# atx/padne

Hardware: AMD Instinct MI355X
Metric: CG solves/s (higher is better)
Workload: dtype f64

## Files before the change

padne_amd/csrc/amg.hip:

```cpp
#include "common.hpp"

#include <functional>
#include <type_traits>
#include <memory>

#include <algorithm>
#include <chrono>
#include <math.h>
#include <stdlib.h>
#include <string.h>

namespace padne {

struct AmgLevel {
    const padne_csr *A = nullptr;
    padne_csr *A_owned = nullptr;
    padne_csr *P = nullptr;
    padne_csr *R = nullptr;
    padne_csr *W = nullptr;
    double lambda = 2.0;
    double jac = 0.0;
    long long n = 0;
    double *b = nullptr, *xa = nullptr, *xb = nullptr, *tmp = nullptr;
    float *b8 = nullptr, *xa8 = nullptr, *xb8 = nullptr, *tmp8 = nullptr;
// ... 18 lines not shown
    int *seg_off = nullptr;
    double *coarse_gather = nullptr;
    double *tail_r = nullptr, *tail_z = nullptr;
    int *tail_slot_idx = nullptr;
    double setup_seconds = 0.0;
    double operator_complexity = 0.0;
    int device = 0;
};

constexpr double kTheta = 0.08;
constexpr double kOmegaNum = 1.5;
constexpr double kChebRatio = 10.0;
constexpr int kLanczosSteps = 8;
constexpr int kMaxLevels = 16;

struct __attribute__((packed, aligned(4))) I4u { int x, y, z, w; };
struct __attribute__((packed, aligned(4))) I2u { int x, y; };
struct __attribute__((packed, aligned(4))) D2u { double x, y; };
struct __attribute__((packed, aligned(4))) L2u { long long x, y; };
__device__ __forceinline__ int4 load_i4_unaligned(const int *p) {
    const I4u v = *reinterpret_cast<const I4u *>(p);
    return make_int4(v.x, v.y, v.z, v.w);
}
__device__ __forceinline__ double2 load_d2_unaligned(const double *p) {
    const D2u v = *reinterpret_cast<const D2u *>(p);
    return make_double2(v.x, v.y);
}

template <int LANES>
__device__ __forceinline__ int scan_incl_lanes(int x) {
    x += __builtin_amdgcn_update_dpp(0, x, 0x111, 0xf, 0xf, false);
    x += __builtin_amdgcn_update_dpp(0, x, 0x112, 0xf, 0xf, false);
    x += __builtin_amdgcn_update_dpp(0, x, 0x114, 0xf, 0xf, false);
    x += __builtin_amdgcn_update_dpp(0, x, 0x118, 0xf, 0xf, false);
    if (LANES >= 32) x += __builtin_amdgcn_update_dpp(0, x, 0x142, 0xa, 0xf, false);
    if (LANES == 64) x += __builtin_amdgcn_update_dpp(0, x, 0x143, 0xc, 0xf, false);
    return x;
}

__device__ __forceinline__ unsigned xcd_bid() {
    const unsigned b = blockIdx.x, per = gridDim.x >> 3;
    if (b >= (per << 3)) return b;
    return (b & 7u) * per + (b >> 3);
}
struct XcdSweep { long long t0, t1, stride; };
__device__ __forceinline__ XcdSweep xcd_sweep(const long long n_tiles, const int waves_per_block, const int w) {
    const unsigned G = gridDim.x;
    const unsigned nslab = (G % kNumXcd == 0) ? kNumXcd : 1;
    const unsigned slab = blockIdx.x % nslab;
    XcdSweep sw;
    const long long s0 = (long long)slab * n_tiles / nslab;
    sw.t1 = (long long)(slab + 1) * n_tiles / nslab;
    sw.t0 = s0 + (long long)(blockIdx.x / nslab) * waves_per_block + w;
    sw.stride = (long long)(G / nslab) * waves_per_block;
    return sw;
}



constexpr unsigned int kMisRoot = 0xffffffffu;
__device__ __forceinline__ unsigned int prio32_of(int i) {
    unsigned int h = (unsigned int)i & 0x7fffffffu;
    h = (h * 0x5bd1e995u) & 0x7fffffffu;
    h ^= h >> 15;
    h = (h * 0x2c1b3c6du) & 0x7fffffffu;
    h ^= h >> 13;
    h = (h * 0x297a2d39u) & 0x7fffffffu;
    h ^= h >> 16;
    return h + 1u;
}

__device__ __forceinline__ bool strong(double a, double di, double dj, double theta2) {
    return a * a * di * dj >= theta2;
}

__device__ __forceinline__ int xw_position(const int4 d, const int run, const int c) {
    int pos = 0;
    if (c >= d.z && c < d.z + run) pos = 2 * run + (c - d.z);
    if (c >= d.y && c < d.y + run) pos = run + (c - d.y);
    if (c >= d.x && c < d.x + run) pos = c - d.x;
    return pos;
}

__global__ __launch_bounds__(256) void strength_mark(int n, int n_wtiles, const int *__restrict__ rowptr,
                                                     const int *__restrict__ cols, const double *__restrict__ vals,
                                                     const double *__restrict__ dinv, double theta2,
                                                     int *__restrict__ scol, double *__restrict__ bound_partial,
                                                     const int4 *__restrict__ xw_desc = nullptr,
                                                     const unsigned char *__restrict__ xw_lidx = nullptr,
                                                     const int xw_run = 0, unsigned char *__restrict__ spos = nullptr,
                                                     float *__restrict__ vals32 = nullptr) {
    constexpr int CH = 512;
    __shared__ unsigned char rid_all[4 * CH];
    __shared__ double pv_all[4 * CH];
    __shared__ double red[4], red2[4];
    const int lane = threadIdx.x & 63, w = threadIdx.x >> 6;
    unsigned char *rid = rid_all + w * CH;
    double *pv = pv_all + w * CH;
    const XcdSweep sw = xcd_sweep(n_wtiles, 4, w);
    double my_max = 0.0, my_plain = 0.0;
    for (long long wt = sw.t0; wt < sw.t1; wt += sw.stride) {
        const int row0 = (int)wt * 64;
        const int row1 = min(row0 + 64, n);
        const int r = row0 + lane;
        int rs = 0, re = 0;
        double di = 0.0;
        if (r < row1) {
            rs = rowptr[r];
            re = rowptr[r + 1];
            di = dinv[r];
        }
        const int k0 = __shfl(rs, 0, 64);
        const int k1 = __shfl(re, row1 - row0 - 1, 64);
        double dF = r < row1 ? 1.0 / di : 1.0, off_strong = 0.0, off_all = 0.0, abs_all = 0.0;
        int4 dsc = make_int4(0, 0, 0, 0);
        if (spos != nullptr) dsc = xw_desc[wt];
        const bool windowed = spos != nullptr && dsc.w != 0;
        const int self_pos = windowed ? xw_position(dsc, xw_run, r) : 0;
        for (int base = k0; base < k1; base += CH) {
            const int lo = max(rs, base), hi = min(re, base + CH);
            for (int k = lo; k < hi; ++k) rid[k - base] = (unsigned char)lane;
            asm volatile("s_waitcnt lgkmcnt(0)" ::: "memory");
            __builtin_amdgcn_wave_barrier();
#pragma unroll
            for (int q = 0; q < CH / 64; ++q) {
                const int e = base + lane + 64 * q;
                const int rl = e < k1 ? rid[e - base] : 0;
                const double dr = __shfl(di, rl, 64);
                const int sp = __shfl(self_pos, rl, 64);
                if (e < k1) {
                    const int i = row0 + rl;
                    const int c = cols[e];
                    const double v = vals[e];
                    if (vals32 != nullptr) vals32[e] = (float)v;
                    const bool st = c != i && strong(v, dr, dinv[c], theta2);
                    scol[e] = st ? c : i;
                    if (windowed) spos[e] = st ? xw_lidx[e] : (unsigned char)sp;
                    if (bound_partial != nullptr) {
                        rid[e - base] = (unsigned char)(rl | (c == i ? 0x40 : 0) | (st ? 0x80 : 0));
                        pv[e - base] = v;
                    }
                }
            }
            if (bound_partial != nullptr) {
                asm volatile("s_waitcnt lgkmcnt(0)" ::: "memory");
                __builtin_amdgcn_wave_barrier();
                for (int k = lo; k < hi; ++k) {
                    const unsigned char f = rid[k - base];
                    const double v = pv[k - base];
                    abs_all += fabs(v);
                    if (f & 0x40) continue;
                    off_all += fabs(v);
                    if (f & 0x80) off_strong += fabs(v);
                    else dF += v;
                }
            }
            asm volatile("" ::: "memory");
            __builtin_amdgcn_wave_barrier();
        }
        if (bound_partial != nullptr && r < row1) {
            double off = off_strong;
            if (!(dF * di > 0.05)) {
                dF = 1.0 / di;
                off = off_all;
            }
            const double sgm = (off + fabs(dF)) / fabs(dF);
            my_max = sgm > my_max ? sgm : my_max;
            const double plain = abs_all * fabs(di);
            my_plain = plain > my_plain ? plain : my_plain;
        }
    }
    if (bound_partial != nullptr) {
        for (int o = 32; o > 0; o >>= 1) {
            my_max = fmax(my_max, __shfl_down(my_max, o, 64));
            my_plain = fmax(my_plain, __shfl_down(my_plain, o, 64));
        }
        if (lane == 0) {
            red[w] = my_max;
            red2[w] = my_plain;
        }
        __syncthreads();
        if (threadIdx.x == 0) {
            bound_partial[blockIdx.x] = fmax(fmax(red[0], red[1]), fmax(red[2], red[3]));
            bound_partial[kMaxPartials + blockIdx.x] = fmax(fmax(red2[0], red2[1]), fmax(red2[2], red2[3]));
        }
    }
}

template <typename T>
__global__ __launch_bounds__(256) void nbr_max(int n, int n_wtiles, const int *__restrict__ srow,
                                               const int *__restrict__ scol, const T *__restrict__ in,
                                               T *__restrict__ out) {
    constexpr int CH = 512;
    __shared__ T park_all[4 * CH];
    const int lane = threadIdx.x & 63, w = threadIdx.x >> 6;
    T *park = park_all + w * CH;
    const XcdSweep sw = xcd_sweep(n_wtiles, 4, w);
    for (long long wt = sw.t0; wt < sw.t1; wt += sw.stride) {
        const int row0 = (int)wt * 64;
        const int row1 = min(row0 + 64, n);
        const int r = row0 + lane;
        int rs = 0, re = 0;
        T m = 0;
        if (r < row1) {
            rs = srow[r];
            re = srow[r + 1];
            m = in[r];
        }
        const int k0 = __shfl(rs, 0, 64);
        const int k1 = __shfl(re, row1 - row0 - 1, 64);
        for (int base = k0; base < k1; base += CH) {
#pragma unroll
            for (int j = 0; j < CH / 64; ++j) {
                const int e = base + lane + 64 * j;
                park[lane + 64 * j] = (e < k1) ? in[scol[e]] : (T)0;
            }
            asm volatile("s_waitcnt lgkmcnt(0)" ::: "memory");
            __builtin_amdgcn_wave_barrier();
            const int lo = max(rs, base), hi = min(re, base + CH);
            for (int k = lo; k < hi; ++k) {
                const T v = park[k - base];
                m = v > m ? v : m;
            }
            asm volatile("" ::: "memory");
            __builtin_amdgcn_wave_barrier();
        }
        if (r < row1) out[r] = m;
    }
}

template <typename T>
__global__ __launch_bounds__(256) void nbr_max_wpr(int n, const int *__restrict__ srow, const int *__restrict__ scol,
                                                   const T *__restrict__ in, T *__restrict__ out) {
    const int lane = threadIdx.x & 63;
    const long long r = (long long)blockIdx.x * 4 + (threadIdx.x >> 6);
    if (r >= n) return;
    const int rs = srow[r], re = srow[r + 1];
    T m = in[r];
    for (int k = rs + lane; k < re; k += 64) {
        const T v = in[scol[k]];
        m = v > m ? v : m;
    }
#pragma unroll
    for (int off = 32; off > 0; off >>= 1) {
        const T o = __shfl_down(m, off, 64);
        m = o > m ? o : m;
    }
    if (lane == 0) out[r] = m;
}

__device__ __forceinline__ bool mis_decide_one(int i, unsigned int top, unsigned int *__restrict__ word,
                                               signed char *__restrict__ state) {
    const unsigned int mine = word[i];
    if (top == kMisRoot) {
        state[i] = 2;
        word[i] = 0u;
        return false;
    }
    if (top == mine) {
        state[i] = 1;
        word[i] = kMisRoot;
        return false;
    }
    return true;
}

template <typename T, bool DECIDE>
__global__ __launch_bounds__(256) void nbr_max_xw(int n, int n_wtiles, const int *__restrict__ srow,
                                                  const int *__restrict__ scol, const unsigned char *__restrict__ spos,
                                                  const int4 *__restrict__ xw_desc, const int run,
                                                  const T *__restrict__ in, T *__restrict__ out,
                                                  unsigned int *__restrict__ word, signed char *__restrict__ state,
                                                  int *__restrict__ undecided) {
    constexpr int CH = 512;
    __shared__ int open_red[4];
    int open = 0;
    __shared__ T park_all[4 * CH];
    __shared__ T xs_all[4 * 3 * 88];
    const int lane = threadIdx.x & 63, w = threadIdx.x >> 6;
    T *park = park_all + w * CH;
    T *xs = xs_all + w * 3 * 88;
    const XcdSweep sw = xcd_sweep(n_wtiles, 4, w);
    for (long long wt = sw.t0; wt < sw.t1; wt += sw.stride) {
        const int row0 = (int)wt * 64;
        const int row1 = min(row0 + 64, n);
        const int r = row0 + lane;
        int rs = 0, re = 0;
        T m = 0;
        if (r < row1) {
            rs = srow[r];
            re = srow[r + 1];
            m = in[r];
        }
        const int4 d = xw_desc[wt];
        const int k0 = __shfl(rs, 0, 64);
        const int k1 = __shfl(re, row1 - row0 - 1, 64);
        if (d.w != 0) {
            const int st[3] = {d.x, d.y, d.z};
#pragma unroll
            for (int q = 0; q < 3; ++q) {
                const int a = st[q] + lane, b = st[q] + 64 + lane;
                xs[q * run + lane] = a < n ? in[a] : (T)0;
                if (lane < run - 64) xs[q * run + 64 + lane] = b < n ? in[b] : (T)0;
            }
            const int top = 3 * run - 1;
            for (int base = k0 & ~3; base < k1; base += CH) {
                unsigned int cw[2];
#pragma unroll
                for (int j = 0; j < 2; ++j) {
                    const int e = base + 4 * lane + 256 * j;
                    cw[j] = e < k1 ? *reinterpret_cast<const unsigned int *>(spos + e) : 0u;
                }
                asm volatile("s_waitcnt lgkmcnt(0)" ::: "memory");
                __builtin_amdgcn_wave_barrier();
#pragma unroll
                for (int j = 0; j < 2; ++j)
#pragma unroll
                    for (int t = 0; t < 4; ++t) park[4 * lane + 256 * j + t] = xs[min((int)((cw[j] >> (8 * t)) & 255u), top)];
                asm volatile("s_waitcnt lgkmcnt(0)" ::: "memory");
                __builtin_amdgcn_wave_barrier();
                const int lo = max(rs, base), hi = min(re, base + CH);
                for (int k = lo; k < hi; ++k) {
                    const T v = park[k - base];
                    m = v > m ? v : m;
                }
                asm volatile("" ::: "memory");
                __builtin_amdgcn_wave_barrier();
            }
        } else {
            for (int base = k0; base < k1; base += CH) {
#pragma unroll
                for (int j = 0; j < CH / 64; ++j) {
                    const int e = base + lane + 64 * j;
                    park[lane + 64 * j] = (e < k1) ? in[scol[e]] : (T)0;
                }
                asm volatile("s_waitcnt lgkmcnt(0)" ::: "memory");
                __builtin_amdgcn_wave_barrier();
                const int lo = max(rs, base), hi = min(re, base + CH);
                for (int k = lo; k < hi; ++k) {
                    const T v = park[k - base];
                    m = v > m ? v : m;
                }
                asm volatile("" ::: "memory");
                __builtin_amdgcn_wave_barrier();
            }
        }
        if (r < row1) {
            if (DECIDE) {
                if (state[r] == 0 && mis_decide_one(r, (unsigned int)m, word, state)) ++open;
            } else {
                out[r] = m;
            }
        }
    }
    if (DECIDE) {
        for (int off = 32; off > 0; off >>= 1) open += __shfl_down(open, off, 64);
        if (lane == 0) open_red[w] = open;
        __syncthreads();
        if (threadIdx.x == 0) {
            const int t = open_red[0] + open_red[1] + open_red[2] + open_red[3];
            if (t) atomicAdd(undecided, t);
        }
    }
}

__global__ void mis_init_words(int n, unsigned int *__restrict__ word, signed char *__restrict__ state,
                               int *__restrict__ counters, int n_counters, unsigned char *__restrict__ pad, int n_pad) {
    const int i = blockIdx.x * blockDim.x + threadIdx.x;
    if (i < n) {
        word[i] = prio32_of(i);
        state[i] = 0;
    }
    if (i < n_counters) counters[i] = 0;
    if (pad != nullptr && i < n_pad) pad[i] = 0;
}

constexpr int kMisTailCap = 512;
__global__ __launch_bounds__(1024) void mis_tail_rounds(const int *__restrict__ cnt_ptr, int *list_a, int *list_b,
                                                        const int *__restrict__ srow, const int *__restrict__ scol,
                                                        unsigned int *word, signed char *state, unsigned int *m2,
                                                        int *__restrict__ count_out, const int max_rounds) {
    __shared__ int s_next;
    int cnt = *cnt_ptr;
    if (threadIdx.x == 0) s_next = 0;
    __syncthreads();
    const int q = threadIdx.x & 7, slot = threadIdx.x >> 3;
    for (int round = 0; round < max_rounds && cnt > 0; ++round) {
        for (int t0 = 0; t0 < cnt; t0 += 128) {
            const int t = t0 + slot;
            const bool live = t < cnt;
            unsigned int m = 0u;
            if (live) {
                const int i = list_a[t];
                m = word[i];
                const int a1 = srow[i + 1];
                for (int a = srow[i] + q; a < a1; a += 8) {
                    const int j = scol[a];
                    if (j == i) continue;
                    const unsigned int wj = word[j];
                    m = wj > m ? wj : m;
                    for (int b = srow[j]; b < srow[j + 1]; ++b) {
                        const unsigned int wk = word[scol[b]];
                        m = wk > m ? wk : m;
                    }
                }
            }
#pragma unroll
            for (int d = 1; d < 8; d <<= 1) {
                const unsigned int o = (unsigned int)__shfl_xor((int)m, d, 64);
                m = o > m ? o : m;
            }
            if (live && q == 0) m2[t] = m;
        }
        __syncthreads();
        for (int t = threadIdx.x; t < cnt; t += 1024) {
            const int i = list_a[t];
            if (mis_decide_one(i, m2[t], word, state)) list_b[atomicAdd(&s_next, 1)] = i;
        }
        __syncthreads();
        cnt = s_next;
        __syncthreads();
        if (threadIdx.x == 0) s_next = 0;
        int *tmp = list_a;
        list_a = list_b;
        list_b = tmp;
        __syncthreads();
    }
    if (threadIdx.x == 0) *count_out = cnt;
}

__global__ __launch_bounds__(256) void mis_decide(int n, unsigned int *__restrict__ word, const unsigned int *__restrict__ m2,
                                                  signed char *__restrict__ state, int *__restrict__ undecided) {
// ... 1573 lines not shown

__global__ __launch_bounds__(256) void fold_max2_kernel(const double *__restrict__ a, const double *__restrict__ b, int g,
                                                        double *__restrict__ out2) {
    __shared__ double red[2][256];
    double ma = 0.0, mb = 0.0;
    for (int q = threadIdx.x; q < g; q += 256) {
        ma = a[q] > ma ? a[q] : ma;
        if (b != nullptr) mb = b[q] > mb ? b[q] : mb;
    }
    red[0][threadIdx.x] = ma;
    red[1][threadIdx.x] = mb;
    __syncthreads();
    for (int off = 128; off > 0; off >>= 1) {
        if ((int)threadIdx.x < off) {
            red[0][threadIdx.x] = fmax(red[0][threadIdx.x], red[0][threadIdx.x + off]);
            red[1][threadIdx.x] = fmax(red[1][threadIdx.x], red[1][threadIdx.x + off]);
        }
        __syncthreads();
    }
    if (threadIdx.x == 0) {
        out2[0] = red[0][0];
        out2[1] = red[1][0];
    }
}

static int gershgorin(padne_ctx *ctx, const padne_csr *A, double *lambda, bool filtered = false) {
    const int g = (int)std::min<long long>((A->n_rows + 255) / 256, 1024);
    double *part = ctx->partials + 6 * kMaxPartials;
    if (filtered)
        hipLaunchKernelGGL(gershgorin_filtered_kernel, dim3(g > 0 ? g : 1), dim3(256), 0, ctx->stream, (int)A->n_rows,
                           A->rowptr, A->cols, A->vals, A->dinv, kTheta * kTheta, part);
    else
        hipLaunchKernelGGL(gershgorin_kernel, dim3(g > 0 ? g : 1), dim3(256), 0, ctx->stream, (int)A->n_rows, A->rowptr,
                           A->vals, A->dinv, part);
    hipLaunchKernelGGL(fold_max2_kernel, dim3(1), dim3(256), 0, ctx->stream, (const double *)part, (const double *)nullptr,
                       g > 0 ? g : 1, part + kMaxPartials - 2);
    PADNE_HIP_CHECK(hipGetLastError());
    double h[2] = {0.0, 0.0};
    PADNE_TRY(read_back(ctx, part + kMaxPartials - 2, sizeof(h), h));
    double m = h[0];
    if (!(m > 0.0) || !(m < 1e6)) m = 2.0;
    *lambda = m;
    return PADNE_OK;
}

static int aggregate(padne_ctx *ctx, Scratch &sc, const padne_csr *A, int **agg_out, int *n_agg, double *lambda_f = nullptr,
                     double *lambda_plain = nullptr, unsigned char **spos_out = nullptr, int **scol_out = nullptr,
                     float *vals32_out = nullptr) {
    hipStream_t s = ctx->stream;
    const int n = (int)A->n_rows;
    const double theta2 = kTheta * kTheta;
    signed char *state = nullptr;
    unsigned int *w0 = nullptr, *w1 = nullptr, *w2 = nullptr;
    int *flag = nullptr, *scan = nullptr, *agg0 = nullptr, *agg1 = nullptr, *counter = nullptr;
    PADNE_TRY(sc.alloc(&state, (size_t)n));
    PADNE_TRY(sc.alloc(&w0, (size_t)n));
    PADNE_TRY(sc.alloc(&w1, (size_t)n));
    PADNE_TRY(sc.alloc(&w2, (size_t)n));
    PADNE_TRY(sc.alloc(&flag, (size_t)n + 1));
    PADNE_TRY(sc.alloc(&scan, (size_t)n + 1));
    PADNE_TRY(sc.alloc(&agg0, (size_t)n));
    PADNE_TRY(sc.alloc(&agg1, (size_t)n));
    constexpr int kMaxRounds = 256;
    PADNE_TRY(sc.alloc(&counter, (size_t)2 * kMaxRounds + 4));
    const dim3 g(nblk(n)), b(256);
    const int *srow = A->rowptr;
    int *scol = nullptr;
    PADNE_TRY(sc.alloc(&scol, (size_t)(A->nnz > 0 ? A->nnz : 1)));
    const int n_wt = (n + 63) / 64;
    int gm_x = std::min(2048, (n_wt + 3) / 4 > 0 ? (n_wt + 3) / 4 : 1);
    if (gm_x >= kNumXcd) gm_x -= gm_x % kNumXcd;
    const dim3 gm((unsigned)gm_x);
    double *bound_part = lambda_f != nullptr ? ctx->partials + 6 * kMaxPartials : nullptr;
    double *bound2 = nullptr;
    if (lambda_f != nullptr) PADNE_TRY(sc.alloc(&bound2, 2));
    const bool xw = A->xw_state == 1 && A->xw_run <= 85;
    unsigned char *spos = nullptr;
    if (xw) {
        PADNE_TRY(sc.alloc(&spos, (size_t)A->nnz + kPadNnz));
    }
    static_assert(kPadNnz >= 2 * kMaxRounds + 4, "one grid for everything the start clears");
    hipLaunchKernelGGL(mis_init_words, dim3(nblk(std::max(n, kPadNnz))), b, 0, s, n, w0, state, counter, 2 * kMaxRounds + 4,
                       spos != nullptr ? spos + A->nnz : (unsigned char *)nullptr, kPadNnz);
    hipLaunchKernelGGL(strength_mark, gm, b, 0, s, n, n_wt, A->rowptr, A->cols, A->vals, A->dinv, theta2, scol, bound_part,
                       xw ? A->xw_desc : (const int4 *)nullptr, xw ? (const unsigned char *)A->xw_lidx : (const unsigned char *)nullptr,
                       xw ? A->xw_run : 0, spos, vals32_out);
    PADNE_HIP_CHECK(hipGetLastError());
    const bool long_rows = !xw && n <= 65536 && A->nnz >= 24LL * n;
    auto launch_round = [&](int *open_counter) {
        if (xw) {
            hipLaunchKernelGGL((nbr_max_xw<unsigned int, false>), gm, b, 0, s, n, n_wt, srow, scol, spos, A->xw_desc, A->xw_run,
                               (const unsigned int *)w0, w1, (unsigned int *)nullptr, (signed char *)nullptr, (int *)nullptr);
            hipLaunchKernelGGL((nbr_max_xw<unsigned int, true>), gm, b, 0, s, n, n_wt, srow, scol, spos, A->xw_desc, A->xw_run,
                               (const unsigned int *)w1, (unsigned int *)nullptr, w0, state, open_counter);
        } else if (long_rows) {
            hipLaunchKernelGGL(nbr_max_wpr<unsigned int>, dim3((unsigned)((n + 3) / 4)), b, 0, s, n, srow, (const int *)scol,
                               (const unsigned int *)w0, w1);
            hipLaunchKernelGGL(nbr_max_wpr<unsigned int>, dim3((unsigned)((n + 3) / 4)), b, 0, s, n, srow, (const int *)scol,
                               (const unsigned int *)w1, w2);
            hipLaunchKernelGGL(mis_decide, dim3(std::min<unsigned>(g.x, 1024u)), b, 0, s, n, w0, w2, state, open_counter);
        } else {
            hipLaunchKernelGGL(nbr_max<unsigned int>, gm, b, 0, s, n, n_wt, srow, scol, w0, w1);
            hipLaunchKernelGGL(nbr_max<unsigned int>, gm, b, 0, s, n, n_wt, srow, scol, w1, w2);
            hipLaunchKernelGGL(mis_decide, dim3(std::min<unsigned>(g.x, 1024u)), b, 0, s, n, w0, w2, state, open_counter);
        }
    };
    if (lambda_f != nullptr)
        hipLaunchKernelGGL(fold_max2_kernel, dim3(1), dim3(256), 0, s, (const double *)bound_part,
                           (const double *)(bound_part + kMaxPartials), (int)gm.x, bound2);
    double h_bound2[2] = {0.0, 0.0};
    bool bound_pending = lambda_f != nullptr;
    auto count_back = [&](const int *dev_count, int *host_count) -> int {
        if (!bound_pending) return read_back(ctx, dev_count, sizeof(int), host_count);
        bound_pending = false;
        return read_back2(ctx, dev_count, sizeof(int), host_count, bound2, sizeof(h_bound2), h_bound2);
    };
    int open_count = n;
    int round = 0;
    const bool compact_ok = A->nnz <= 16LL * n;
    const int full_batch = n > 200000 ? 1 : 4;
    while (round < kMaxRounds && open_count > 0 && (!compact_ok || round < 2 || open_count > n / 8)) {
        const int reps = (round == 0 && compact_ok && full_batch < 2) ? 2 : full_batch;
        for (int rep = 0; rep < reps && round < kMaxRounds; ++rep, ++round) {
            launch_round(counter + round);
        }
        PADNE_HIP_CHECK(hipGetLastError());
        PADNE_TRY(count_back(counter + round - 1, &open_count));
    }
    if (open_count > 0) {
        int *list_a = (int *)w1, *list_b = (int *)w2;
        unsigned int *m2 = nullptr;
        PADNE_TRY(sc.alloc(&m2, (size_t)open_count));
        int *counters = counter + kMaxRounds;
        hipLaunchKernelGGL(mis_collect_open, dim3(std::min<unsigned>(g.x, 1024u)), b, 0, s, n, state, list_a, counters);
        PADNE_HIP_CHECK(hipGetLastError());
        int cnt = open_count, cur = 0;
        while (cur + 1 < kMaxRounds && cnt > 0) {
            if (cnt <= kMisTailCap) {
                hipLaunchKernelGGL(mis_tail_rounds, dim3(1), dim3(1024), 0, s, (const int *)(counters + cur), list_a, list_b, srow,
                                   (const int *)scol, w0, state, m2, counters + cur + 1, kMaxRounds - cur - 1);
                PADNE_HIP_CHECK(hipGetLastError());
                ++cur;
                round += kMaxRounds;
                PADNE_TRY(count_back(counters + cur, &cnt));
                break;
            }
            const dim3 gl(nblk(cnt));
            const int batch = 4;
            for (int rep = 0; rep < batch && cur + 1 < kMaxRounds; ++rep, ++round) {
                hipLaunchKernelGGL(mis_two_hop_max, dim3(nblk((long long)cnt * kHopLanes)), b, 0, s, counters + cur, list_a, srow, scol, w0, m2);
                hipLaunchKernelGGL(mis_decide_list, gl, b, 0, s, counters + cur, list_a, m2, w0, state, list_b, counters + cur + 1);
                std::swap(list_a, list_b);
                ++cur;
            }
            PADNE_HIP_CHECK(hipGetLastError());
            PADNE_TRY(count_back(counters + cur, &cnt));
        }
        open_count = cnt;
    }
    PADNE_REQUIRE(open_count == 0, "independent-set rounds did not terminate");
    if (lambda_f != nullptr) {
        if (bound_pending) PADNE_TRY(read_back(ctx, bound2, sizeof(h_bound2), h_bound2));
        double m = h_bound2[0], mp = h_bound2[1];
        if (!(m > 0.0) || !(m < 1e6)) m = 2.0;
        if (!(mp > 0.0) || !(mp < 1e6)) mp = 2.0;
        *lambda_f = m;
        if (lambda_plain != nullptr) *lambda_plain = mp;
    }
    hipLaunchKernelGGL(flag_state, g, b, 0, s, n, state, flag, 1);
    ScanTicket t_roots, t_single;
    long long h_roots[2] = {0, 0}, h_single[2] = {0, 0};
    PADNE_TRY(scan_i32_begin(ctx, flag, scan, n, &t_roots, true));
    hipLaunchKernelGGL(agg_from_roots, g, b, 0, s, n, state, scan, agg0);
    hipLaunchKernelGGL(agg_join, g, b, 0, s, n, srow, scol, A->vals, agg0, agg1);
    hipLaunchKernelGGL(agg_join, g, b, 0, s, n, srow, scol, A->vals, agg1, agg0);
    hipLaunchKernelGGL(flag_unaggregated, g, b, 0, s, n, agg0, flag);
    int rc_scan = scan_i32_begin(ctx, flag, scan, n, &t_single, true);
// ... 1987 lines not shown
```

padne_amd/csrc/capi.hip:

```cpp
#include "common.hpp"

#include <algorithm>

#include <math.h>
#include <stdarg.h>
#include <string.h>
#include <chrono>

namespace padne {

std::atomic<long long> g_launch_count{0};

void options_from_env(padne_options *o) {
    *o = padne_options();
    auto on = [](const char *name) { const char *e = getenv(name); return e != nullptr && e[0] != '\0' && !(e[0] == '0' && e[1] == '\0'); };
    auto has = [](const char *list, const char *word) {
        const size_t n = strlen(word);
        for (const char *p = list; p != nullptr && *p != '\0';) {
            const char *q = strchr(p, ',');
            const size_t len = q != nullptr ? (size_t)(q - p) : strlen(p);
            if (len >= n && strncmp(p, word, n) == 0 && (len == n || p[n] == ':')) return p;
            p = q != nullptr ? q + 1 : nullptr;
        }
        return (const char *)nullptr;
    };
    o->amg_f64 = on("PADNE_AMG_F64");
    if (const char *e = getenv("PADNE_AMG_W")) o->amg_w = strcmp(e, "none") == 0 ? 0 : (strcmp(e, "fine") == 0 ? 1 : 2);
    o->amg_exchange_all = on("PADNE_AMG_EXCHANGE_ALL");
    o->pcg_p64 = on("PADNE_PCG_P64");
    o->pcg_no_xhist = on("PADNE_PCG_NO_XHIST");
    o->gj_vector = on("PADNE_GJ_VECTOR");
    o->no_batch = on("PADNE_NO_BATCH");
    o->no_mailbox = on("PADNE_NO_MAILBOX");
    o->no_p2p = on("PADNE_NO_P2P");
    o->no_split = on("PADNE_NO_SPLIT");
    o->no_xwindow = on("PADNE_NO_XWINDOW");
    o->setup_one_stream = on("PADNE_SETUP_ONE_STREAM");
    if (const char *e = getenv("PADNE_CG_SINGLE_REDUCTION")) o->cg_single_reduction = atoi(e) != 0 ? 1 : 0;
    if (const char *e = getenv("PADNE_LOCKSTEP_NARROW")) o->lockstep_narrow = atoi(e);
    if (const char *e = getenv("PADNE_AMG_COARSE_N")) o->amg_coarse_n = std::min(4096, std::max(16, atoi(e)));
    if (const char *e = getenv("PADNE_AMG_GATHER_N")) o->amg_gather_n = atoll(e);
    if (const char *e = getenv("PADNE_P2P_TIMEOUT_MS")) {
        const long v = atol(e);
        if (v > 0 && v <= 600000) o->p2p_timeout_ms = (unsigned)v;
    }
    if (const char *f = getenv("PADNE_FORCE")) {
        o->force_asm_hash = has(f, "asm_hash") != nullptr;
        o->force_asm_two_pass = has(f, "asm_two_pass") != nullptr;
        o->force_relabel_slots = has(f, "relabel_slots") != nullptr;
        o->force_transpose_cursors = has(f, "transpose_cursors") != nullptr;
        o->force_xhist_small = has(f, "xhist_small") != nullptr;
        o->force_relabel_lanes = has(f, "relabel_lanes") != nullptr;
        if (const char *w = has(f, "spgemm_split")) o->force_spgemm_split = w[12] == ':' ? atoll(w + 13) : 30000;
    }
    if (const char *v = getenv("PADNE_VERBOSE")) {
        o->verbose_amg = has(v, "amg") != nullptr;
        o->verbose_xw = has(v, "xw") != nullptr;
        o->verbose_pool = has(v, "pool") != nullptr;
    }
}

static thread_local char g_err[1024] = "";

void set_error(const char *fmt, ...) {
    va_list ap;
    va_start(ap, fmt);
    vsnprintf(g_err, sizeof(g_err), fmt, ap);
    va_end(ap);
}

int ensure_workspace(padne_ctx *ctx, size_t bytes) {
    if (ctx->ws_bytes >= bytes) return PADNE_OK;
    if (ctx->ws) {
        PADNE_HIP_CHECK(hipStreamSynchronize(ctx->stream));
        PADNE_HIP_CHECK(hipFree(ctx->ws));
        ctx->ws = nullptr;
        ctx->ws_bytes = 0;
    }
    if (hipMalloc(&ctx->ws, bytes) != hipSuccess) {
        set_error("hipMalloc of %zu workspace bytes failed", bytes);
        return PADNE_E_NOMEM;
    }
    ctx->ws_bytes = bytes;
    return PADNE_OK;
}

constexpr size_t kPoolCacheLimit = (size_t)240 << 30;

static size_t pool_round(size_t bytes) {
    if (bytes < 256) bytes = 256;
    if (bytes >= ((size_t)1 << 20)) return (bytes + ((size_t)1 << 20) - 1) & ~(((size_t)1 << 20) - 1);
    size_t p = 256;
    while (p < bytes) p <<= 1;
    return p;
}

void *pool_alloc(padne_ctx *ctx, size_t bytes) {
    const size_t want = pool_round(bytes);
    auto it = ctx->pool_free_blocks.lower_bound(want);
    if (it != ctx->pool_free_blocks.end() && it->first <= want + want / 2 + ((size_t)1 << 20)) {
        void *p = it->second;
        ctx->pool_cached_bytes -= it->first;
        ctx->pool_free_blocks.erase(it);
        return p;
    }
    void *p = nullptr;
    const bool trace = ctx->opt.verbose_pool;
    if (trace) fprintf(stderr, "[pool] %s hipMalloc %zu bytes (cached %zu)\n", ctx->is_aux ? "aux" : "main", want, ctx->pool_cached_bytes);
    hipError_t e = hipMalloc(&p, want);
    if (e != hipSuccess) {
        (void)hipGetLastError();
        pool_release_all(ctx);
        e = hipMalloc(&p, want);
    }
    if (e != hipSuccess) {
        (void)hipGetLastError();
        set_error("hipMalloc of %zu bytes failed: %s", want, hipGetErrorString(e));
        return nullptr;
    }
    ctx->pool_sizes[p] = want;
    return p;
}

void pool_free(padne_ctx *ctx, void *p) {
    if (p == nullptr) return;
    auto it = ctx->pool_sizes.find(p);
    if (it == ctx->pool_sizes.end()) {
        padne_ctx *other = ctx->is_aux ? ctx->parent : ctx->aux;
        if (other != nullptr && other->pool_sizes.count(p)) {
            pool_free(other, p);
            return;
        }
        (void)hipFree(p);
        return;
    }
// ... 497 lines not shown
```

padne_amd/csrc/common.hpp:

```cpp
#pragma once

#include <hip/hip_runtime.h>
#include <stdint.h>
#include <stdio.h>
#include <map>
#include <string>
#include <unordered_map>
#include <vector>

#include "../../include/padne_hip.h"
#include "../../include/padne_hip_test.h"
#include "../../include/padne_hip_probe.h"

#include <atomic>

namespace padne {

extern std::atomic<long long> g_launch_count;

void set_error(const char *fmt, ...);

#define PADNE_HIP_CHECK(expr)                                                              \
    do {                                                                                   \
        hipError_t _e = (expr);                                                            \
// ... 12 lines not shown
        }                                                                                  \
    } while (0)

#define PADNE_TRY(...)                                                                     \
    do {                                                                                   \
        int _rc = (__VA_ARGS__);                                                           \
        if (_rc != PADNE_OK) return _rc;                                                   \
    } while (0)

}
#undef hipLaunchKernelGGL
#define hipLaunchKernelGGL(kernelName, numBlocks, numThreads, memPerBlock, streamId, ...)   \
    do {                                                                                   \
        ::padne::g_launch_count.fetch_add(1, std::memory_order_relaxed);                   \
        kernelName<<<(numBlocks), (numThreads), (memPerBlock), (streamId)>>>(__VA_ARGS__); \
    } while (0)
#define hipMemsetAsync(...) (::padne::g_launch_count.fetch_add(1, std::memory_order_relaxed), hipMemsetAsync(__VA_ARGS__))
namespace padne {

constexpr int kNumXcd = 8;

constexpr int kSpmvThreads = 256;
constexpr int kSpmvRows = 256;
constexpr int kPadNnz = 4096;

constexpr int kMaxPartials = 2048;
constexpr int kPinnedSlots = 16;
constexpr int kPinnedSlotBase = 4096;
constexpr int kPinnedBytes = kPinnedSlotBase + 512 * kPinnedSlots;

constexpr int kTinySystem = 32;
constexpr int kSpmmK = 8;

}

struct padne_csr {
    int64_t n_rows = 0, n_cols = 0, nnz = 0;
    int32_t *rowptr = nullptr;
    int32_t *cols = nullptr;
    double *vals = nullptr;
    double *dinv = nullptr;
    int device = 0;
    padne_ctx *owner = nullptr;
    void *amg = nullptr;
    float *vals32 = nullptr, *dinv32 = nullptr;
    int4 *xw_desc = nullptr;
    unsigned short *xw_lidx = nullptr;
    int xw_state = 0;
    int xw_run = 0;
    int xw_nruns = 3;
    int *split_tiles = nullptr;
    int split_n_int = 0, split_n_bnd = 0;
    int split_state = 0;
    bool hierarchy_operator = false;
    bool cols_unsorted = false;
    padne_csr *prec_block = nullptr;
    double *mesh_xy = nullptr, *mesh_sigma = nullptr;
    int32_t *mesh_tri = nullptr;
    long long *mesh_voff = nullptr, *mesh_toff = nullptr;
    int64_t mesh_n_vert = 0, mesh_n_tri = 0, mesh_n_mesh = 0;
};

struct padne_options {
    bool amg_f64 = false;
    int amg_w = 2;
    bool amg_exchange_all = false;
    bool pcg_p64 = false;
    bool pcg_no_xhist = false;
    bool gj_vector = false;
    bool no_batch = false;
    bool no_mailbox = false;
    bool no_p2p = false;
    bool no_split = false;
    bool no_xwindow = false;
    bool setup_one_stream = false;
    int cg_single_reduction = -1;
    int lockstep_narrow = -1;
    int amg_coarse_n = 2048;
    long long amg_gather_n = 0;
    unsigned p2p_timeout_ms = 20000;
    bool force_asm_hash = false, force_asm_two_pass = false, force_relabel_slots = false, force_transpose_cursors = false;
    bool force_relabel_lanes = false;
    bool force_xhist_small = false;
    long long force_spgemm_split = 0;
    bool verbose_amg = false, verbose_xw = false, verbose_pool = false;
};
namespace padne { void options_from_env(padne_options *o); }

struct padne_ctx {
    int device = 0;
    padne_options opt;
    hipStream_t stream = nullptr;
    double *partials = nullptr;
    double *scalars = nullptr;
    int32_t *status = nullptr;
    void *pinned = nullptr;
    void *ws = nullptr;
    size_t ws_bytes = 0;
    void *comm = nullptr;
    void *team = nullptr;
    int rank = 0, world = 1;
    bool halo_on = false;
    long long halo_n_owned = 0;
    int halo_m = 0, halo_n_export = 0;
    int32_t *halo_export = nullptr;
    void *p2p_mbox = nullptr;
    void **p2p_peers = nullptr;
    int p2p_m_cap = 0;
    unsigned long long p2p_seq = 0;
    bool p2p_ipc = false;
    std::vector<void *> p2p_ipc_mapped;
    unsigned p2p_timeout_ms = 20000;
    int (*hostcoll_fn)(void *, const void *, void *, int64_t) = nullptr;
    void *hostcoll_user = nullptr;
    hipEvent_t ev0 = nullptr, ev1 = nullptr;
    hipStream_t copy_stream[4] = {nullptr, nullptr, nullptr, nullptr};
    padne_ctx *aux = nullptr, *parent = nullptr;
    bool is_aux = false;
    unsigned long long lockstep_groups = 0;
    unsigned pinned_busy = 0;
    unsigned long long *mailbox = nullptr, *mailbox_dev = nullptr;
    unsigned long long mail_seq = 0;
    hipEvent_t ev_order = nullptr;
    std::multimap<size_t, void *> pool_free_blocks;
    std::unordered_map<void *, size_t> pool_sizes;
    size_t pool_cached_bytes = 0;
};

namespace padne {

int ensure_workspace(padne_ctx *ctx, size_t bytes);
int csr_alloc(padne_ctx *ctx, int64_t n_rows, int64_t n_cols, int64_t nnz, padne_csr **out);
int csr_shrink_nnz(padne_ctx *ctx, padne_csr *m, int64_t nnz);
int csr_build_dinv(padne_ctx *ctx, padne_csr *m);

int spmv_grid(const padne_csr *m);
enum { SPMV_PLAIN = 0, SPMV_DOT = 1, SPMV_RESID = 2, SPMV_ADD = 3, SPMV_JACOBI = 4,
       SPMV_DOT_AUX = 5,
       SPMV_WUP = 6,
       SPMV_RESTRICT = 7,
       SPMV_RESID_PRE = 8 };
enum { SPMV_ALL = 0, SPMV_INTERIOR = 1, SPMV_BOUNDARY = 2 };

template <typename XT> struct ProductArgs {
    const XT *b = nullptr;
    const XT *dinv = nullptr;
    XT scale = 0;
    const XT *x_pre = nullptr;
    XT *y2 = nullptr;
    const XT *rhs = nullptr;
    const double *dot_with = nullptr;
    double *partials = nullptr;
    const double *out_scale2 = nullptr;
    const int32_t *done_flag = nullptr;
};
template <typename XT> inline const XT *product_vals(const padne_csr *m) {
    if constexpr (sizeof(XT) == 4) return m->vals32;
    else return m->vals;
}

template <typename XT, typename YT, typename ST = XT>
int launch_spmv(padne_ctx *ctx, const padne_csr *m, int mode, const ST *x, YT *y, const ProductArgs<XT> &a, int part = SPMV_ALL);
template <typename XT, typename YT>
int launch_spmm(padne_ctx *ctx, const padne_csr *m, int k, int mode, const XT *x, YT *y, const ProductArgs<XT> &a);
inline int launch_spmv(padne_ctx *ctx, const padne_csr *m, const double *x, double *y, const double *dot_with, double *partials,
                       const int32_t *done_flag) {
// ... 126 lines not shown
```

Baseline: 31.42.

## Prefetch next tile headers and vectorize strength marking in AMG setup kernels

The strength_mark and nbr_max_xw kernels now load the next wave-tile's row pointers, diagonal, window descriptor and MIS state/word while the current tile is processed, hiding global load latency across the tile loop. strength_mark also processes edges in groups of four with int4/double2/float4 vector loads and stores instead of one element per lane. The old serial path is kept behind a PADNE_FORCE=serial_tiles option. This adds register pressure, and the vectorized path assumes edge arrays are aligned to groups of four from a rounded-down base. It only affects AMG setup, which may be a small share of per-solve time.

```diff
diff --git a/padne_amd/csrc/amg.hip b/padne_amd/csrc/amg.hip
--- a/padne_amd/csrc/amg.hip
+++ b/padne_amd/csrc/amg.hip
@@ -124,6 +124,7 @@
     return pos;
 }
 
+template <bool PIPE = true>
 __global__ __launch_bounds__(256) void strength_mark(int n, int n_wtiles, const int *__restrict__ rowptr,
                                                      const int *__restrict__ cols, const double *__restrict__ vals,
                                                      const double *__restrict__ dinv, double theta2,
@@ -141,46 +142,128 @@
     double *pv = pv_all + w * CH;
     const XcdSweep sw = xcd_sweep(n_wtiles, 4, w);
     double my_max = 0.0, my_plain = 0.0;
+    int rs_n = 0, re_n = 0;
+    double di_n = 0.0;
+    int4 dsc_n = make_int4(0, 0, 0, 0);
+    auto fetch_head = [&](const long long wt) {
+        const int r = (int)wt * 64 + lane;
+        rs_n = re_n = 0;
+        di_n = 0.0;
+        if (wt < sw.t1) {
+            if (spos != nullptr) dsc_n = xw_desc[wt];
+            if (r < n) {
+                rs_n = rowptr[r];
+                re_n = rowptr[r + 1];
+                di_n = dinv[r];
+            }
+        }
+    };
+    if (PIPE) fetch_head(sw.t0);
     for (long long wt = sw.t0; wt < sw.t1; wt += sw.stride) {
         const int row0 = (int)wt * 64;
         const int row1 = min(row0 + 64, n);
         const int r = row0 + lane;
         int rs = 0, re = 0;
         double di = 0.0;
-        if (r < row1) {
-            rs = rowptr[r];
-            re = rowptr[r + 1];
-            di = dinv[r];
+        int4 dsc = make_int4(0, 0, 0, 0);
+        if (PIPE) {
+            rs = rs_n;
+            re = re_n;
+            di = di_n;
+            dsc = dsc_n;
+            fetch_head(wt + sw.stride);
+        } else {
+            if (r < row1) {
+                rs = rowptr[r];
+                re = rowptr[r + 1];
+                di = dinv[r];
+            }
+            if (spos != nullptr) dsc = xw_desc[wt];
         }
         const int k0 = __shfl(rs, 0, 64);
         const int k1 = __shfl(re, row1 - row0 - 1, 64);
         double dF = r < row1 ? 1.0 / di : 1.0, off_strong = 0.0, off_all = 0.0, abs_all = 0.0;
-        int4 dsc = make_int4(0, 0, 0, 0);
-        if (spos != nullptr) dsc = xw_desc[wt];
         const bool windowed = spos != nullptr && dsc.w != 0;
         const int self_pos = windowed ? xw_position(dsc, xw_run, r) : 0;
-        for (int base = k0; base < k1; base += CH) {
+        for (int base = PIPE ? (k0 & ~3) : k0; base < k1; base += CH) {
             const int lo = max(rs, base), hi = min(re, base + CH);
             for (int k = lo; k < hi; ++k) rid[k - base] = (unsigned char)lane;
-            asm volatile("s_waitcnt lgkmcnt(0)" ::: "memory");
-            __builtin_amdgcn_wave_barrier();
-#pragma unroll
-            for (int q = 0; q < CH / 64; ++q) {
-                const int e = base + lane + 64 * q;
-                const int rl = e < k1 ? rid[e - base] : 0;
-                const double dr = __shfl(di, rl, 64);
-                const int sp = __shfl(self_pos, rl, 64);
-                if (e < k1) {
-                    const int i = row0 + rl;
-                    const int c = cols[e];
-                    const double v = vals[e];
-                    if (vals32 != nullptr) vals32[e] = (float)v;
-                    const bool st = c != i && strong(v, dr, dinv[c], theta2);
-                    scol[e] = st ? c : i;
-                    if (windowed) spos[e] = st ? xw_lidx[e] : (unsigned char)sp;
-                    if (bound_partial != nullptr) {
-                        rid[e - base] = (unsigned char)(rl | (c == i ? 0x40 : 0) | (st ? 0x80 : 0));
-                        pv[e - base] = v;
+            if (PIPE) {
+                constexpr int G = 4;
+                asm volatile("s_waitcnt lgkmcnt(0)" ::: "memory");
+                __builtin_amdgcn_wave_barrier();
+#pragma unroll 1
+                for (int e0 = base + G * lane; e0 < base + CH; e0 += 64 * G) {
+                    int4 cw = make_int4(0, 0, 0, 0);
+                    double2 va = make_double2(0.0, 0.0), vb = make_double2(0.0, 0.0);
+                    unsigned int lw = 0u;
+                    if (e0 < k1) {
+                        cw = *reinterpret_cast<const int4 *>(cols + e0);
+                        va = *reinterpret_cast<const double2 *>(vals + e0);
+                        vb = *reinterpret_cast<const double2 *>(vals + e0 + 2);
+                        if (windowed) lw = *reinterpret_cast<const unsigned int *>(xw_lidx + e0);
+                    }
+                    const int c[G] = {cw.x, cw.y, cw.z, cw.w};
+                    const double v[G] = {va.x, va.y, vb.x, vb.y};
+                    double dc[G];
+#pragma unroll
+                    for (int t = 0; t < G; ++t) dc[t] = (e0 + t >= k0 && e0 + t < k1) ? dinv[c[t]] : 0.0;
+                    int sc_[G], rl[G];
+                    unsigned int sp_w = 0u;
+#pragma unroll
+                    for (int t = 0; t < G; ++t) rl[t] = (e0 + t >= k0 && e0 + t < k1) ? rid[e0 + t - base] : 0;
+#pragma unroll
+                    for (int t = 0; t < G; ++t) {
+                        const double dr = __shfl(di, rl[t], 64);
+                        const int sp = __shfl(self_pos, rl[t], 64);
+                        const int i = row0 + rl[t];
+                        const bool st = c[t] != i && strong(v[t], dr, dc[t], theta2);
+                        sc_[t] = st ? c[t] : i;
+                        sp_w |= (st ? (lw >> (8 * t)) & 255u : (unsigned int)(sp & 255)) << (8 * t);
+                        const int e = e0 + t;
+                        if (bound_partial != nullptr && e >= k0 && e < k1) {
+                            rid[e - base] = (unsigned char)(rl[t] | (c[t] == i ? 0x40 : 0) | (st ? 0x80 : 0));
+                            pv[e - base] = v[t];
+                        }
+                    }
+                    if (e0 >= k0 && e0 + G <= k1) {
+                        *reinterpret_cast<int4 *>(scol + e0) = make_int4(sc_[0], sc_[1], sc_[2], sc_[3]);
+                        if (windowed) *reinterpret_cast<unsigned int *>(spos + e0) = sp_w;
+                        if (vals32 != nullptr)
+                            *reinterpret_cast<float4 *>(vals32 + e0) = make_float4((float)v[0], (float)v[1], (float)v[2], (float)v[3]);
+                    } else if (e0 < k1) {
+#pragma unroll
+                        for (int t = 0; t < G; ++t) {
+                            const int e = e0 + t;
+                            if (e >= k0 && e < k1) {
+                                scol[e] = sc_[t];
+                                if (windowed) spos[e] = (unsigned char)(sp_w >> (8 * t));
+                                if (vals32 != nullptr) vals32[e] = (float)v[t];
+                            }
+                        }
+                    }
+                }
+            } else {
+                asm volatile("s_waitcnt lgkmcnt(0)" ::: "memory");
+                __builtin_amdgcn_wave_barrier();
+#pragma unroll
+                for (int q = 0; q < CH / 64; ++q) {
+                    const int e = base + lane + 64 * q;
+                    const int rl = e < k1 ? rid[e - base] : 0;
+                    const double dr = __shfl(di, rl, 64);
+                    const int sp = __shfl(self_pos, rl, 64);
+                    if (e < k1) {
+                        const int i = row0 + rl;
+                        const int c = cols[e];
+                        const double v = vals[e];
+                        if (vals32 != nullptr) vals32[e] = (float)v;
+                        const bool st = c != i && strong(v, dr, dinv[c], theta2);
+                        scol[e] = st ? c : i;
+                        if (windowed) spos[e] = st ? xw_lidx[e] : (unsigned char)sp;
+                        if (bound_partial != nullptr) {
+                            rid[e - base] = (unsigned char)(rl | (c == i ? 0x40 : 0) | (st ? 0x80 : 0));
+                            pv[e - base] = v;
+                        }
                     }
                 }
             }
@@ -307,7 +390,22 @@
     return true;
 }
 
-template <typename T, bool DECIDE>
+__device__ __forceinline__ bool mis_decide_own(int i, unsigned int top, unsigned int mine, unsigned int *__restrict__ word,
+                                               signed char *__restrict__ state) {
+    if (top == kMisRoot) {
+        state[i] = 2;
+        word[i] = 0u;
+        return false;
+    }
+    if (top == mine) {
+        state[i] = 1;
+        word[i] = kMisRoot;
+        return false;
+    }
+    return true;
+}
+
+template <typename T, bool DECIDE, bool PIPE = true>
 __global__ __launch_bounds__(256) void nbr_max_xw(int n, int n_wtiles, const int *__restrict__ srow,
                                                   const int *__restrict__ scol, const unsigned char *__restrict__ spos,
                                                   const int4 *__restrict__ xw_desc, const int run,
@@ -323,18 +421,56 @@
     T *park = park_all + w * CH;
     T *xs = xs_all + w * 3 * 88;
     const XcdSweep sw = xcd_sweep(n_wtiles, 4, w);
+    int rs_n = 0, re_n = 0;
+    T m_n = 0;
+    int4 d_n = make_int4(0, 0, 0, 0);
+    signed char st_n = 1;
+    unsigned int wd_n = 0u;
+    auto fetch_head = [&](const long long wt) {
+        const int r = (int)wt * 64 + lane;
+        rs_n = re_n = 0;
+        m_n = 0;
+        st_n = 1;
+        wd_n = 0u;
+        if (wt < sw.t1) {
+            d_n = xw_desc[wt];
+            if (r < n) {
+                rs_n = srow[r];
+                re_n = srow[r + 1];
+                m_n = in[r];
+                if (DECIDE) {
+                    st_n = state[r];
+                    wd_n = word[r];
+                }
+            }
+        }
+    };
+    if (PIPE) fetch_head(sw.t0);
     for (long long wt = sw.t0; wt < sw.t1; wt += sw.stride) {
         const int row0 = (int)wt * 64;
         const int row1 = min(row0 + 64, n);
         const int r = row0 + lane;
         int rs = 0, re = 0;
         T m = 0;
-        if (r < row1) {
-            rs = srow[r];
-            re = srow[r + 1];
-            m = in[r];
-        }
-        const int4 d = xw_desc[wt];
+        int4 d;
+        signed char st_r = 1;
+        unsigned int wd_r = 0u;
+        if (PIPE) {
+            rs = rs_n;
+            re = re_n;
+            m = m_n;
+            d = d_n;
+            st_r = st_n;
+            wd_r = wd_n;
+            fetch_head(wt + sw.stride);
+        } else {
+            if (r < row1) {
+                rs = srow[r];
+                re = srow[r + 1];
+                m = in[r];
+            }
+            d = xw_desc[wt];
+        }
         const int k0 = __shfl(rs, 0, 64);
         const int k1 = __shfl(re, row1 - row0 - 1, 64);
         if (d.w != 0) {
@@ -389,7 +525,11 @@
         }
         if (r < row1) {
             if (DECIDE) {
-                if (state[r] == 0 && mis_decide_one(r, (unsigned int)m, word, state)) ++open;
+                if (PIPE) {
+                    if (st_r == 0 && mis_decide_own(r, (unsigned int)m, wd_r, word, state)) ++open;
+                } else {
+                    if (state[r] == 0 && mis_decide_one(r, (unsigned int)m, word, state)) ++open;
+                }
             } else {
                 out[r] = m;
             }
@@ -2129,17 +2269,20 @@
     static_assert(kPadNnz >= 2 * kMaxRounds + 4, "one grid for everything the start clears");
     hipLaunchKernelGGL(mis_init_words, dim3(nblk(std::max(n, kPadNnz))), b, 0, s, n, w0, state, counter, 2 * kMaxRounds + 4,
                        spos != nullptr ? spos + A->nnz : (unsigned char *)nullptr, kPadNnz);
-    hipLaunchKernelGGL(strength_mark, gm, b, 0, s, n, n_wt, A->rowptr, A->cols, A->vals, A->dinv, theta2, scol, bound_part,
-                       xw ? A->xw_desc : (const int4 *)nullptr, xw ? (const unsigned char *)A->xw_lidx : (const unsigned char *)nullptr,
-                       xw ? A->xw_run : 0, spos, vals32_out);
+    const bool serial = ctx->opt.force_serial_tiles;
+    hipLaunchKernelGGL((serial ? strength_mark<false> : strength_mark<true>), gm, b, 0, s, n, n_wt, A->rowptr, A->cols, A->vals,
+                       A->dinv, theta2, scol, bound_part, xw ? A->xw_desc : (const int4 *)nullptr,
+                       xw ? (const unsigned char *)A->xw_lidx : (const unsigned char *)nullptr, xw ? A->xw_run : 0, spos, vals32_out);
     PADNE_HIP_CHECK(hipGetLastError());
     const bool long_rows = !xw && n <= 65536 && A->nnz >= 24LL * n;
     auto launch_round = [&](int *open_counter) {
         if (xw) {
-            hipLaunchKernelGGL((nbr_max_xw<unsigned int, false>), gm, b, 0, s, n, n_wt, srow, scol, spos, A->xw_desc, A->xw_run,
-                               (const unsigned int *)w0, w1, (unsigned int *)nullptr, (signed char *)nullptr, (int *)nullptr);
-            hipLaunchKernelGGL((nbr_max_xw<unsigned int, true>), gm, b, 0, s, n, n_wt, srow, scol, spos, A->xw_desc, A->xw_run,
-                               (const unsigned int *)w1, (unsigned int *)nullptr, w0, state, open_counter);
+            hipLaunchKernelGGL((serial ? nbr_max_xw<unsigned int, false, false> : nbr_max_xw<unsigned int, false, true>), gm, b, 0, s,
+                               n, n_wt, srow, scol, spos, A->xw_desc, A->xw_run, (const unsigned int *)w0, w1, (unsigned int *)nullptr,
+                               (signed char *)nullptr, (int *)nullptr);
+            hipLaunchKernelGGL((serial ? nbr_max_xw<unsigned int, true, false> : nbr_max_xw<unsigned int, true, true>), gm, b, 0, s,
+                               n, n_wt, srow, scol, spos, A->xw_desc, A->xw_run, (const unsigned int *)w1, (unsigned int *)nullptr,
+                               w0, state, open_counter);
         } else if (long_rows) {
             hipLaunchKernelGGL(nbr_max_wpr<unsigned int>, dim3((unsigned)((n + 3) / 4)), b, 0, s, n, srow, (const int *)scol,
                                (const unsigned int *)w0, w1);
diff --git a/padne_amd/csrc/capi.hip b/padne_amd/csrc/capi.hip
--- a/padne_amd/csrc/capi.hip
+++ b/padne_amd/csrc/capi.hip
@@ -51,6 +51,7 @@
         o->force_transpose_cursors = has(f, "transpose_cursors") != nullptr;
         o->force_xhist_small = has(f, "xhist_small") != nullptr;
         o->force_relabel_lanes = has(f, "relabel_lanes") != nullptr;
+        o->force_serial_tiles = has(f, "serial_tiles") != nullptr;
         if (const char *w = has(f, "spgemm_split")) o->force_spgemm_split = w[12] == ':' ? atoll(w + 13) : 30000;
     }
     if (const char *v = getenv("PADNE_VERBOSE")) {
diff --git a/padne_amd/csrc/common.hpp b/padne_amd/csrc/common.hpp
--- a/padne_amd/csrc/common.hpp
+++ b/padne_amd/csrc/common.hpp
@@ -118,6 +118,7 @@
     bool force_asm_hash = false, force_asm_two_pass = false, force_relabel_slots = false, force_transpose_cursors = false;
     bool force_relabel_lanes = false;
     bool force_xhist_small = false;
+    bool force_serial_tiles = false;
     long long force_spgemm_split = 0;
     bool verbose_amg = false, verbose_xw = false, verbose_pool = false;
 };
```

New measurement: 31.76, median of 6. Within noise of the previous version (+1.1%).
